# tlog-dev/eazy

Measured on AMD Instinct MI355X. Metric: device-resident compress+decompress GiB/s, 1 MiB block, 1/2/4/8 MI355X, higher is better.
Workload: dtype u8

## Files before the change

### eazy_amd/csrc/ez_k1_lean.hip

```cpp
#include "ez_k1_internal.h"

#include <cstdio>
#include <cstring>
#include <algorithm>
#include <vector>

namespace ez {
namespace {
using namespace k1;

struct GWU {
    const uint8_t *p;
    __device__ __forceinline__ void around(int32_t y, uint64_t &before, uint64_t &from) const {
        V16 v = ld16v(p + (y - 8));
        if (y < 8) {
            const int32_t k = 8 - y;
            v.lo &= k >= 8 ? 0ull : ~0ull << (8 * k);
            v.hi &= k >= 16 ? 0ull : (k <= 8 ? ~0ull : ~0ull << (8 * (k - 8)));
        }
        before = v.lo;
        from = v.hi;
    }
};

template <int R = 80, int G = 16>
struct WinLds {
    static constexpr int LB = 128 / G;
    typedef unsigned int u32v __attribute__((ext_vector_type(LB / 4)));
    u32v f;
    int32_t cb, fb, bmax, pm;
    uint8_t *wl;
    __device__ __forceinline__ int32_t floor4(int32_t y) const { return y - ((pm + y) & 3); }
    __device__ __forceinline__ void ld(const uint8_t *p, int32_t b, int lj, u32v &d) const {
        typedef const __attribute__((address_space(1))) u32v *gp;
        d = *(gp)(p + b + LB * lj);
    }
    __device__ __forceinline__ void put(int lj) const { *(u32v *)(wl + LB * lj) = f; }
    __device__ __forceinline__ void init(const uint8_t *p, int32_t n, int lj, bool live) {
        pm = (int32_t)((uintptr_t)p & 3);
        bmax = floor4(n - 64);
        cb = min(floor4(-8), bmax);
        fb = min(cb + 64, bmax);
        f = u32v{};
        if (live) ld(p, cb, lj, f);
        put(lj);
        if (live) ld(p, fb, lj, f);
    }
    __device__ __forceinline__ void advance(const uint8_t *p, int32_t i, int lj, bool live) {
        const int32_t y = i - 8;
        if (live && !(y >= cb && y - cb <= R)) {
            if (!(y >= fb && y - fb <= R)) {
                fb = min(floor4(y), bmax);
                ld(p, fb, lj, f);
            }
            cb = fb;
            put(lj);
            fb = min(cb + 64, bmax);
            ld(p, fb, lj, f);
        }
    }
    __device__ __forceinline__ void bytes(int32_t i, int g, int lj, V16 &w0, V16 &w1) const {
        const uint32_t o = (uint32_t)(i - 8 - cb + lj), r = o & 3;
        const uint32_t *q = (const uint32_t *)(wl + (o & ~3u));
        uint32_t d[9];
#pragma unroll
        for (int t = 0; t < 9; t++) d[t] = q[t];
        uint32_t b[8];
#pragma unroll
        for (int t = 0; t < 8; t++) b[t] = __builtin_amdgcn_alignbyte(d[t + 1], d[t], r);
        w0.lo = (uint64_t)b[0] | ((uint64_t)b[1] << 32);
        w0.hi = (uint64_t)b[2] | ((uint64_t)b[3] << 32);
        w1.lo = (uint64_t)b[4] | ((uint64_t)b[5] << 32);
        w1.hi = (uint64_t)b[6] | ((uint64_t)b[7] << 32);
    }
    __device__ __forceinline__ void bytes48(int32_t i, int g, int lj, V16 &w0, V16 &w1, V16 &w2) const {
        static_assert(R <= 64, "48-byte windows need the region to reach i + 54");
        const uint32_t o = (uint32_t)(i - 8 - cb + lj), r = o & 3;
        const uint32_t *q = (const uint32_t *)(wl + (o & ~3u));
        uint32_t d[13];
#pragma unroll
        for (int t = 0; t < 13; t++) d[t] = q[t];
        uint32_t b[12];
#pragma unroll
        for (int t = 0; t < 12; t++) b[t] = __builtin_amdgcn_alignbyte(d[t + 1], d[t], r);
        w0 = V16{(uint64_t)b[0] | ((uint64_t)b[1] << 32), (uint64_t)b[2] | ((uint64_t)b[3] << 32)};
        w1 = V16{(uint64_t)b[4] | ((uint64_t)b[5] << 32), (uint64_t)b[6] | ((uint64_t)b[7] << 32)};
        w2 = V16{(uint64_t)b[8] | ((uint64_t)b[9] << 32), (uint64_t)b[10] | ((uint64_t)b[11] << 32)};
    }
};

__device__ __forceinline__ void bytes32(const LeanIn &L, const uint8_t *p, int32_t y, V16 &c0, V16 &c1) {
    const uintptr_t a = (uintptr_t)(p + y - 8);
    const uint32_t r = (uint32_t)(a & 3);
    const uint8_t *w = (const uint8_t *)(a & ~(uintptr_t)3);
    const uint4 q0 = L.dw4(w), q1 = L.dw4(w + 16);
    const uint32_t q2 = L.dw(w + 32);
    const uint32_t d[9] = {q0.x, q0.y, q0.z, q0.w, q1.x, q1.y, q1.z, q1.w, q2};
    uint32_t b[8];
#pragma unroll
    for (int t = 0; t < 8; t++) b[t] = __builtin_amdgcn_alignbyte(d[t + 1], d[t], r);
    c0.lo = (uint64_t)b[0] | ((uint64_t)b[1] << 32);
    c0.hi = (uint64_t)b[2] | ((uint64_t)b[3] << 32);
    c1.lo = (uint64_t)b[4] | ((uint64_t)b[5] << 32);
    c1.hi = (uint64_t)b[6] | ((uint64_t)b[7] << 32);
}

__device__ __forceinline__ void bytes48(const LeanIn &L, const uint8_t *p, int32_t y, V16 &c0, V16 &c1, V16 &c2) {
    const uintptr_t a = (uintptr_t)(p + y);
    const uint32_t r = (uint32_t)(a & 3);
    const uint8_t *w = (const uint8_t *)(a & ~(uintptr_t)3) - 8;
    const uint4 q0 = L.dw4(w), q1 = L.dw4(w + 16), q2 = L.dw4(w + 32);
    const uint32_t q3 = L.dw(w + 48);
    const uint32_t d[13] = {q0.x, q0.y, q0.z, q0.w, q1.x, q1.y, q1.z, q1.w, q2.x, q2.y, q2.z, q2.w, q3};
    uint32_t b[12];
#pragma unroll
    for (int t = 0; t < 12; t++) b[t] = __builtin_amdgcn_alignbyte(d[t + 1], d[t], r);
    c0 = V16{(uint64_t)b[0] | ((uint64_t)b[1] << 32), (uint64_t)b[2] | ((uint64_t)b[3] << 32)};
    c1 = V16{(uint64_t)b[4] | ((uint64_t)b[5] << 32), (uint64_t)b[6] | ((uint64_t)b[7] << 32)};
    c2 = V16{(uint64_t)b[8] | ((uint64_t)b[9] << 32), (uint64_t)b[10] | ((uint64_t)b[11] << 32)};
}

#if (EZ_EXP & 65536)
__device__ unsigned long long g_lean_hist[18];
#endif

template <int FW, int G>
__device__ __forceinline__ void lean_run(const CompressArgs &A, int lj, int g, uint16_t *hth, uint32_t table_words, uint32_t hsh,
                                         uint64_t *recs, uint64_t rcap, int prio, uint8_t *edge, uint8_t *wl) {
    constexpr int S = 64 / G;
    constexpr uint32_t kGMask = (1u << G) - 1;
    constexpr bool W40 = FW == 40;
    static_assert(FW == 24 || W40, "the judgement's forward cap is 24 or 40 bytes");
    constexpr int32_t CAP = FW;
    const LeanIn L{};
    const uint8_t *blo = A.in, *bhi = A.in + A.in_off[A.count];
    uint32_t *slots = (uint32_t *)(edge + 128 + kEdgeSlots * edge_slot_bytes(A));
    const uint32_t rcap32 = (uint32_t)rcap;

    uint64_t s = (uint64_t)blockIdx.x * S + (uint64_t)g;
    const uint8_t *p = edge + 16;
    int32_t n = 0, i = 0, done = 0, nrec = 0;
    int err = 0;
    bool live = false, pending = false;
    uint64_t *rec = recs;
    V16 z0{0, 0}, z1{0, 0}, z2{0, 0};
    WinLds<W40 ? 64 : 80, G> wr;
    wr.wl = wl;
    int64_t budget = 0;

    auto open = [&]() {
        pending = s < A.count;
        n = 0;
        const uint8_t *src = blo;
        if (pending) {
            n = (int32_t)(A.in_off[s + 1] - A.in_off[s]);
            src = A.in + A.in_off[s];
        }
        for (int32_t k = 4 * lj; k < (int32_t)table_words; k += 4 * G) *(uint4 *)((uint32_t *)hth + k) = make_uint4(0, 0, 0, 0);
        err = !pending || (uint64_t)n > A.max_len ? EZ_EINVAL : 0;
        live = !err && n >= 4;
        p = live ? src : edge + 16;
        const bool edge_stream = live && (src - kEdgeBefore < blo || src + n + 64 > bhi);
        if (edge_stream) {
            int32_t slot = 0;
            if (lj == 0) slot = (int32_t)atomicAdd(slots, 1u);
            slot = bcast(slot, G * g);
            if (slot >= kEdgeSlots) {
                err = EZ_ESTUCK;
                live = false;
                p = edge + 16;
            } else {
                uint8_t *d = edge + 128 + (uint64_t)slot * edge_slot_bytes(A);
                for (int32_t k = lj; k < n + kEdgeBefore + 64; k += G)
                    d[k] = (k >= kEdgeBefore && k < n + kEdgeBefore) ? src[k - kEdgeBefore] : (uint8_t)0;
                p = d + kEdgeBefore;
            }
            __threadfence_block();
        }
        i = done = nrec = 0;
        rec = recs + (pending ? s : 0) * rcap;
        wr.init(p, n, lj, live);
        z0 = z1 = z2 = V16{0, 0};
        if (live) {
            if constexpr (W40) bytes48(L, p, 0, z0, z1, z2);
            else bytes32(L, p, 0, z0, z1);
            z0.lo = 0;
        }
    };
    open();
    budget += (int64_t)(4 * A.max_len + 64) * S;

    V16 w0{0, 0}, w1{0, 0}, w2{0, 0};
    for (;;) {
        if (__builtin_amdgcn_ballot_w64(!live && pending) != 0) {
            if (!live && pending) {
                if (lj == 0) A.out_size[s] = (uint64_t)nrec | ((uint64_t)err << 48);
                pending = false;
            }
        }
        if (__builtin_amdgcn_ballot_w64(live) == 0) break;
        if (budget < 0) {
            if (live) err = EZ_ESTUCK;
            live = false;
            continue;
        }
        const uint64_t lm = __builtin_amdgcn_ballot_w64(live);
        do {
        budget--;
        if constexpr (W40) wr.bytes48(i, g, lj, w0, w1, w2);
        else wr.bytes(i, g, lj, w0, w1);
        const int32_t nvalid = n - 3 - i < G ? n - 3 - i : G;
        const int32_t x = i + lj;
        const bool valid = live && lj < nvalid;

        if (prio & 1) __builtin_amdgcn_s_setprio(3);
        const uint32_t h = valid ? ((uint32_t)w0.hi * kHashMul) >> hsh : 0u;
        int32_t cand = 0;
        if (valid) cand = (int32_t)lds_mskor16(hth, h, (uint32_t)x);
        V16 c0 = z0, c1 = z1, c2 = z2;
        if (cand != 0) {
            if constexpr (W40) bytes48(L, p, cand, c0, c1, c2);
            else bytes32(L, p, cand, c0, c1);
            if (__builtin_expect(cand < 8, 0)) c0.lo &= ~0ull << (8 * (8 - cand));
        }
        if (prio & 1) __builtin_amdgcn_s_setprio(0);

        const bool rl = cand >= done && cand < x;
        const uint64_t e0 = w0.hi ^ c0.hi, e1 = w1.lo ^ c1.lo, e2 = w1.hi ^ c1.hi;
        int32_t jf = W40 ? first_diff40(e0, e1, e2, w2.lo ^ c2.lo, w2.hi ^ c2.hi) : first_diff24(e0, e1, e2);
        jf = jf < n - x ? jf : n - x;
        int32_t bl = x - done;
        if (rl) bl = bl < cand ? bl : cand;
        int32_t jb = last_diff8(w0.lo ^ c0.lo);
        jb = jb < bl ? jb : bl;
        const bool zr = rl && c0.hi == 0 && cand + 8 < n;
        const int32_t fw = rl ? jf : (jf < done - cand ? jf : done - cand);
        const bool acc = valid && (zr || fw + jb >= kMinCopyChunk);

        int32_t lit, nx, dist, ext;
        bool force = false;
        if (zr) {
            int32_t zf = W40 ? first_diff40(0, c1.lo, c1.hi, c2.lo, c2.hi) : first_diff24(0, c1.lo, c1.hi);
            zf = zf < n - cand ? zf : n - cand;
            int32_t zb = last_diff8(c0.lo);
            zb = zb < cand - done ? zb : cand - done;
            lit = cand - zb;
            nx = cand + zf;
            dist = 0;
            ext = (zf == CAP && n - cand > CAP ? 1 : 0) | (zb == 8 && cand - done > 8 ? 2 : 0);
        } else {
            lit = x - jb;
            nx = x + fw;
            dist = x - cand;
            force = rl;
            ext = (jf == CAP && (rl ? n - x : (done - cand < n - x ? done - cand : n - x)) > CAP ? 1 : 0) |
                  (jb == 8 && bl > 8 ? 2 : 0);
        }
        const uint64_t am64 = __builtin_amdgcn_ballot_w64(acc);
        const uint32_t am = (uint32_t)(am64 >> (G * g)) & kGMask;
        const int a = am ? __builtin_ctz(am) : -1;
#if (EZ_EXP & 65536)
        if (live && lj == 0) atomicAdd(&g_lean_hist[a + 1], 1ull);
#endif
        const bool act = live && a >= 0;
        const bool ins1 = !rl && !zr && x + 1 + 4 <= n;
        const int32_t pack = nx | (ext << 28) | ((int32_t)ins1 << 30);
        const int32_t sel = __builtin_amdgcn_ds_bpermute(4 * (G * g + (a < 0 ? 0 : a)), pack);
        int32_t nxt = sel & 0x0fffffff;
        if (__builtin_amdgcn_ballot_w64(act && ((sel >> 28) & 3) != 0) != 0) {
            const int32_t info = cand | (((zr ? cand : x) - lit) << 16) | ((int32_t)rl << 29) | ((int32_t)zr << 30);
            const int32_t ib = bcast(info, G * g + (a < 0 ? 0 : a));
            const int32_t xa = i + (a < 0 ? 0 : a);
            const int32_t ca = ib & 0xffff;
            const bool rla = (ib >> 29) & 1, zra = (ib >> 30) & 1;
            const int32_t e = (sel >> 28) & 3;
            const bool need = act && e != 0;
            const int mode = zra ? 0 : (rla ? 1 : 2);
            const int32_t fa = zra ? ca : xa;
            const int32_t blim = zra ? ca - done : (rla ? ((xa - done) < ca ? (xa - done) : ca) : xa - done);
            const int32_t flim = zra ? n - ca : (rla ? n - xa : ((done - ca) < n - xa ? done - ca : n - xa));
            int32_t fx, cx;
            gext<G, GWU>(GWU{p}, need && (e & 1), need && (e & 2), g, lj, fa, ca, mode, done, CAP, flim, blim, fx, cx);
            if (need) {
                const int32_t f = (e & 1) ? fx : (sel & 0x0fffffff) - fa;
                const int32_t c = (e & 2) ? cx : ((ib >> 16) & 0xf);
                nxt = fa + f;
                if (lj == a) {
                    lit = fa - c;
                    nx = nxt;
                }
            }
        }
        const bool ins_next = (prio & 4) && a >= 0 && a < G - 1 && ((sel >> 30) & 1);
        if (valid && a >= 0 && lj > a && cand <= i + a) hth[h] = (uint16_t)(ins_next && lj == a + 1 ? x : cand);
        if (act && lj == a && !ins_next) {
            if (ins1) {
                const uint32_t h1 = ((uint32_t)(w0.hi >> 8) * kHashMul) >> hsh;
                hth[h1] = (uint16_t)(x + 1);
            }
        }
        const bool st_rec = act && lj == a;
        const uint64_t rv = rec_pack(lit, nx - lit, dist, force);
        const uint32_t rat = (uint32_t)nrec;
        const bool rec_room = (uint32_t)nrec < rcap32;
        if (act) {
            if (!rec_room) { err = EZ_ESTUCK; live = false; }
            nrec++;
            i = done = nxt;
        } else if (live) {
            i += nvalid;
        }
        if (live && (err || i + 4 > n)) live = false;
        wr.advance(p, i, lj, live);
        __builtin_amdgcn_sched_barrier(0);
        if (st_rec && rec_room) __builtin_nontemporal_store(rv, rec + rat);
        } while (__builtin_amdgcn_ballot_w64(live) == lm && budget >= 0);
    }
}


constexpr int kLeanWaves16 = 5;
#if (EZ_EXP & 2097152)
constexpr uint32_t kLeanTMax = 1u << 18;
__device__ uint64_t g_lean_t[2 * kLeanTMax];
#endif
template <int FW, int G>
__global__ __launch_bounds__(64, G == 8 ? 2 : kLeanWaves16) void k1_lean(CompressArgs A, uint32_t stride_words, uint32_t table_words, uint64_t *recs,
                                                                          uint64_t rcap, int prio, uint8_t *edge) {
    constexpr int S = 64 / G;
    extern __shared__ __attribute__((aligned(16))) uint8_t smem[];
    const int lane = (int)(threadIdx.x & 63);
    const int g = lane / G, lj = lane % G;
    const int32_t hs = (int32_t)A.hs;
    const uint32_t hsh = 32u - (uint32_t)(64 - __builtin_clzll((uint64_t)(hs - 1)));
    uint16_t *hth = (uint16_t *)((uint32_t *)smem + (uint32_t)g * stride_words);
    uint8_t *wl = smem + (size_t)4 * stride_words * S + (size_t)g * kWinLdsBytes;
#if (EZ_EXP & 2097152)
    const uint64_t t_start = __builtin_amdgcn_s_memrealtime();
#endif
    lean_run<FW, G>(A, lj, g, hth, table_words, hsh, recs, rcap, prio, edge, wl);
#if (EZ_EXP & 2097152)
    {
        const uint64_t t_end = __builtin_amdgcn_s_memrealtime();
        uint32_t hw = 0, xcc = 0;
        asm volatile("s_getreg_b32 %0, hwreg(HW_REG_HW_ID)" : "=s"(hw));
        asm volatile("s_getreg_b32 %0, hwreg(HW_REG_XCC_ID)" : "=s"(xcc));
        if (lane == 0 && blockIdx.x < kLeanTMax) {
            g_lean_t[2 * blockIdx.x] = t_start;
            g_lean_t[2 * blockIdx.x + 1] = (t_end & 0xffffffffffull) | ((uint64_t)((hw >> 8) & 15) << 40) | ((uint64_t)((hw >> 13) & 7) << 44) |
                                           ((uint64_t)((hw >> 12) & 1) << 47) | ((uint64_t)(xcc & 15) << 48) | ((uint64_t)((hw >> 4) & 3) << 52);
        }
    }
#endif
}

#if (EZ_EXP & 2097152)
void lean_report_timeline(uint64_t blocks, hipStream_t st) {
    const uint64_t nb = blocks < kLeanTMax ? blocks : kLeanTMax;
    std::vector<uint64_t> t(2 * nb);
    (void)hipStreamSynchronize(st);
    (void)hipMemcpyFromSymbol(t.data(), HIP_SYMBOL(g_lean_t), 16 * nb);
    uint64_t t0 = ~0ull, t1 = 0, xe[16] = {0}, xs[16], cnt[16] = {0};
    for (int k = 0; k < 16; k++) xs[k] = ~0ull;
    for (uint64_t b = 0; b < nb; b++) {
        const uint64_t st0 = t[2 * b] & 0xffffffffffull, en = t[2 * b + 1] & 0xffffffffffull;
        const int x = (int)((t[2 * b + 1] >> 48) & 15);
        t0 = st0 < t0 ? st0 : t0;
        t1 = en > t1 ? en : t1;
        xe[x] = en > xe[x] ? en : xe[x];
        xs[x] = st0 < xs[x] ? st0 : xs[x];
        cnt[x]++;
    }
    const int bins = 40;
    std::vector<double> act(bins, 0.0);
    std::vector<uint64_t> ends(nb), lens(nb);
    for (uint64_t b = 0; b < nb; b++) {
        const uint64_t st0 = (t[2 * b] & 0xffffffffffull) - t0, en = (t[2 * b + 1] & 0xffffffffffull) - t0;
        ends[b] = en;
        lens[b] = en - st0;
        for (int k = 0; k < bins; k++) {
            const double lo = (double)(t1 - t0) * k / bins, hi = (double)(t1 - t0) * (k + 1) / bins;
            const double ov = std::min((double)en, hi) - std::max((double)st0, lo);
            if (ov > 0) act[k] += ov / (hi - lo);
        }
    }
    std::sort(ends.begin(), ends.end());
    std::sort(lens.begin(), lens.end());
    fprintf(stderr, "lean waves %llu span %.1f us; wave life p10 %.1f p50 %.1f p90 %.1f max %.1f us; end p50 %.1f p90 %.1f p99 %.1f us\n",
            (unsigned long long)nb, (t1 - t0) / 100.0, lens[nb / 10] / 100.0, lens[nb / 2] / 100.0, lens[nb * 9 / 10] / 100.0, lens[nb - 1] / 100.0,
            ends[nb / 2] / 100.0, ends[nb * 9 / 10] / 100.0, ends[nb * 99 / 100] / 100.0);
    fprintf(stderr, "lean active waves per bin of %.1f us:", (t1 - t0) / 100.0 / bins);
    for (int k = 0; k < bins; k++) fprintf(stderr, " %.0f", act[k]);
    fprintf(stderr, "\nlean per xcc (waves, first start, last end, us):");
    for (int x = 0; x < 16; x++)
        if (cnt[x]) fprintf(stderr, " [%d %llu %.1f %.1f]", x, (unsigned long long)cnt[x], (xs[x] - t0) / 100.0, (xe[x] - t0) / 100.0);
    fprintf(stderr, "\n");
}
#endif
#if (EZ_EXP & 65536)
void lean_report_hist(hipStream_t st) {
    unsigned long long hst[18];
    (void)hipStreamSynchronize(st);
    (void)hipMemcpyFromSymbol(hst, HIP_SYMBOL(g_lean_hist), sizeof hst);
    unsigned long long tot = 0, vis = 0;
    for (int t = 0; t < 18; t++) tot += hst[t];
    for (int t = 1; t < 17; t++) vis += hst[t] * (unsigned long long)t;
    vis += hst[0] * 16ull;
    fprintf(stderr, "lean windows %llu (no accept %llu); visited lanes %.3f of 16; by acceptor lane:", tot, hst[0], (double)vis / (double)tot);
    for (int t = 1; t < 17; t++) fprintf(stderr, " %.3f", (double)hst[t] / (double)tot);
    fprintf(stderr, "\n");
    memset(hst, 0, sizeof hst);
    (void)hipMemcpyToSymbol(HIP_SYMBOL(g_lean_hist), hst, sizeof hst);
}
#endif

template <int FW, int G>
hipError_t launch_lean_v(const CompressArgs &a, uint64_t *recs, uint32_t stride, uint32_t tw, size_t lds, int prio, uint8_t *edge,
                         hipStream_t st) {
    static bool attr_done = false;
    if (!attr_done) {
        (void)hipFuncSetAttribute((const void *)k1_lean<FW, G>, hipFuncAttributeMaxDynamicSharedMemorySize, 160 * 1024);
        attr_done = true;
    }
    constexpr uint64_t S = 64 / G;
    const uint64_t blocks = (a.count + S - 1) / S;
    hipLaunchKernelGGL((k1_lean<FW, G>), dim3((unsigned)blocks), dim3(64), lds, st, a, stride, tw, recs, rec_cap(a), prio, edge);
    return hipGetLastError();
}

}

hipError_t launch_lean(const CompressArgs &a, uint64_t *recs, hipStream_t st) {
    const bool g8 = a.max_len > 4096;
    const bool w40 = a.max_len <= 16384;
    const int S = g8 ? 8 : 4;
    const uint32_t stride = split_stride<16, true>(a), tw = split_table_words<true>(a);
    const uint64_t rcap = rec_cap(a);
    static const int prio = knob("EZ_K1S_PRIO", 1) | (knob("EZ_K1S_NEXT1", 1) ? 4 : 0);
    uint8_t *edge = (uint8_t *)(recs + a.count * rcap);
    hipError_t z = hipMemsetAsync(edge, 0, 128, st);
    if (z == hipSuccess) z = hipMemsetAsync(edge + 128 + kEdgeSlots * edge_slot_bytes(a), 0, 16, st);
    if (z != hipSuccess) return z;
    static const size_t pad = (size_t)knob("EZ_K1S_LDSPAD", 0);
    const size_t lds = (size_t)stride * 4 * S + (size_t)kWinLdsBytes * S + pad;
    hipError_t e;
    const char *route;
    if (!g8) route = "s:lean g16 fw40", e = launch_lean_v<40, 16>(a, recs, stride, tw, lds, prio, edge, st);
    else if (w40) route = "s:lean g8 fw40", e = launch_lean_v<40, 8>(a, recs, stride, tw, lds, prio, edge, st);
    else route = "s:lean g8 fw24", e = launch_lean_v<24, 8>(a, recs, stride, tw, lds, prio, edge, st);
    set_compress_route(route);
    if (e != hipSuccess) return e;
#if (EZ_EXP & 2097152)
    lean_report_timeline((a.count + S - 1) / S, st);
#endif
#if (EZ_EXP & 65536)
    lean_report_hist(st);
#endif
    return launch_emit(a, recs, rcap, false, st);
}

}
```

Baseline: 117.1.

## Add interior fast path to lean match loop without bounds checks

Splits the per-window loop body into a templated lambda with an interior variant used while every lane's group has at least G+CAP-1 bytes left and record room. The interior path drops the end-of-block clamps, the liveness and rcap checks, and simplifies the extension flags to fire whenever a match reaches the cap. This is meant to cut scalar and vector ALU work per window in the common case. It adds a wave-wide ballot per iteration and duplicates the loop body, which raises code size and may raise register pressure. It also changes the ext flags in the boundary path, so more gext calls may fire there and rely on flim/blim to stay correct.

```diff
diff --git a/eazy_amd/csrc/ez_k1_lean.hip b/eazy_amd/csrc/ez_k1_lean.hip
--- a/eazy_amd/csrc/ez_k1_lean.hip
+++ b/eazy_amd/csrc/ez_k1_lean.hip
@@ -3,6 +3,7 @@
 #include <cstdio>
 #include <cstring>
 #include <algorithm>
+#include <type_traits>
 #include <vector>
 
 namespace ez {
@@ -121,7 +122,7 @@
 }
 
 #if (EZ_EXP & 65536)
-__device__ unsigned long long g_lean_hist[18];
+__device__ unsigned long long g_lean_hist[23];
 #endif
 
 template <int FW, int G>
@@ -191,27 +192,17 @@
     budget += (int64_t)(4 * A.max_len + 64) * S;
 
     V16 w0{0, 0}, w1{0, 0}, w2{0, 0};
-    for (;;) {
-        if (__builtin_amdgcn_ballot_w64(!live && pending) != 0) {
-            if (!live && pending) {
-                if (lj == 0) A.out_size[s] = (uint64_t)nrec | ((uint64_t)err << 48);
-                pending = false;
-            }
-        }
-        if (__builtin_amdgcn_ballot_w64(live) == 0) break;
-        if (budget < 0) {
-            if (live) err = EZ_ESTUCK;
-            live = false;
-            continue;
-        }
-        const uint64_t lm = __builtin_amdgcn_ballot_w64(live);
-        do {
+
+    constexpr int32_t kIn = G + CAP - 1;
+
+    auto window = [&](auto in_tag) __attribute__((always_inline)) {
+        constexpr bool IN = decltype(in_tag)::value;
         budget--;
         if constexpr (W40) wr.bytes48(i, g, lj, w0, w1, w2);
         else wr.bytes(i, g, lj, w0, w1);
-        const int32_t nvalid = n - 3 - i < G ? n - 3 - i : G;
+        const int32_t nvalid = IN ? G : (n - 3 - i < G ? n - 3 - i : G);
         const int32_t x = i + lj;
-        const bool valid = live && lj < nvalid;
+        const bool valid = IN || (live && lj < nvalid);
 
         if (prio & 1) __builtin_amdgcn_s_setprio(3);
         const uint32_t h = valid ? ((uint32_t)w0.hi * kHashMul) >> hsh : 0u;
@@ -228,12 +219,12 @@
         const bool rl = cand >= done && cand < x;
         const uint64_t e0 = w0.hi ^ c0.hi, e1 = w1.lo ^ c1.lo, e2 = w1.hi ^ c1.hi;
         int32_t jf = W40 ? first_diff40(e0, e1, e2, w2.lo ^ c2.lo, w2.hi ^ c2.hi) : first_diff24(e0, e1, e2);
-        jf = jf < n - x ? jf : n - x;
+        if constexpr (!IN) jf = jf < n - x ? jf : n - x;
         int32_t bl = x - done;
         if (rl) bl = bl < cand ? bl : cand;
         int32_t jb = last_diff8(w0.lo ^ c0.lo);
         jb = jb < bl ? jb : bl;
-        const bool zr = rl && c0.hi == 0 && cand + 8 < n;
+        const bool zr = rl && c0.hi == 0 && (IN || cand + 8 < n);
         const int32_t fw = rl ? jf : (jf < done - cand ? jf : done - cand);
         const bool acc = valid && (zr || fw + jb >= kMinCopyChunk);
 
@@ -241,29 +232,29 @@
         bool force = false;
         if (zr) {
             int32_t zf = W40 ? first_diff40(0, c1.lo, c1.hi, c2.lo, c2.hi) : first_diff24(0, c1.lo, c1.hi);
-            zf = zf < n - cand ? zf : n - cand;
+            if constexpr (!IN) zf = zf < n - cand ? zf : n - cand;
             int32_t zb = last_diff8(c0.lo);
             zb = zb < cand - done ? zb : cand - done;
             lit = cand - zb;
             nx = cand + zf;
             dist = 0;
-            ext = (zf == CAP && n - cand > CAP ? 1 : 0) | (zb == 8 && cand - done > 8 ? 2 : 0);
+            ext = (zf == CAP ? 1 : 0) | (zb == 8 ? 2 : 0);
         } else {
             lit = x - jb;
             nx = x + fw;
             dist = x - cand;
             force = rl;
-            ext = (jf == CAP && (rl ? n - x : (done - cand < n - x ? done - cand : n - x)) > CAP ? 1 : 0) |
-                  (jb == 8 && bl > 8 ? 2 : 0);
+            ext = (jf == CAP ? 1 : 0) | (jb == 8 ? 2 : 0);
         }
         const uint64_t am64 = __builtin_amdgcn_ballot_w64(acc);
         const uint32_t am = (uint32_t)(am64 >> (G * g)) & kGMask;
         const int a = am ? __builtin_ctz(am) : -1;
 #if (EZ_EXP & 65536)
-        if (live && lj == 0) atomicAdd(&g_lean_hist[a + 1], 1ull);
-#endif
-        const bool act = live && a >= 0;
-        const bool ins1 = !rl && !zr && x + 1 + 4 <= n;
+        if ((IN || live) && lj == 0) atomicAdd(&g_lean_hist[a + 1], 1ull);
+        if (lj == 0 && g == 0) atomicAdd(&g_lean_hist[21], 1ull);
+#endif
+        const bool act = (IN || live) && a >= 0;
+        const bool ins1 = !rl && !zr && (IN || x + 1 + 4 <= n);
         const int32_t pack = nx | (ext << 28) | ((int32_t)ins1 << 30);
         const int32_t sel = __builtin_amdgcn_ds_bpermute(4 * (G * g + (a < 0 ? 0 : a)), pack);
         int32_t nxt = sel & 0x0fffffff;
@@ -280,6 +271,11 @@
             const int32_t blim = zra ? ca - done : (rla ? ((xa - done) < ca ? (xa - done) : ca) : xa - done);
             const int32_t flim = zra ? n - ca : (rla ? n - xa : ((done - ca) < n - xa ? done - ca : n - xa));
             int32_t fx, cx;
+#if (EZ_EXP & 65536)
+            if (need && lj == 0) atomicAdd(&g_lean_hist[18 + ((e & 1 && flim > CAP) || (e & 2 && blim > 8) ? 0 : 1)], 1ull);
+            if (lj == 0 && g == 0) atomicAdd(&g_lean_hist[20], 1ull);
+            if (__builtin_amdgcn_ballot_w64(need && ((e & 1 && flim > CAP) || (e & 2 && blim > 8))) != 0 && lj == 0 && g == 0) atomicAdd(&g_lean_hist[22], 1ull);
+#endif
             gext<G, GWU>(GWU{p}, need && (e & 1), need && (e & 2), g, lj, fa, ca, mode, done, CAP, flim, blim, fx, cx);
             if (need) {
                 const int32_t f = (e & 1) ? fx : (sel & 0x0fffffff) - fa;
@@ -302,18 +298,45 @@
         const bool st_rec = act && lj == a;
         const uint64_t rv = rec_pack(lit, nx - lit, dist, force);
         const uint32_t rat = (uint32_t)nrec;
-        const bool rec_room = (uint32_t)nrec < rcap32;
+        const bool rec_room = IN || (uint32_t)nrec < rcap32;
         if (act) {
             if (!rec_room) { err = EZ_ESTUCK; live = false; }
             nrec++;
             i = done = nxt;
-        } else if (live) {
+        } else if (IN || live) {
             i += nvalid;
         }
-        if (live && (err || i + 4 > n)) live = false;
-        wr.advance(p, i, lj, live);
+        if constexpr (!IN) {
+            if (live && (err || i + 4 > n)) live = false;
+        }
+        wr.advance(p, i, lj, IN || live);
         __builtin_amdgcn_sched_barrier(0);
         if (st_rec && rec_room) __builtin_nontemporal_store(rv, rec + rat);
+    };
+
+    for (;;) {
+        if (__builtin_amdgcn_ballot_w64(!live && pending) != 0) {
+            if (!live && pending) {
+                if (lj == 0) A.out_size[s] = (uint64_t)nrec | ((uint64_t)err << 48);
+                pending = false;
+            }
+        }
+        if (__builtin_amdgcn_ballot_w64(live) == 0) break;
+        if (budget < 0) {
+            if (live) err = EZ_ESTUCK;
+            live = false;
+            continue;
+        }
+        if (__builtin_amdgcn_ballot_w64(live && i + kIn <= n && (uint32_t)nrec < rcap32) == ~0ull) {
+            do {
+                window(std::true_type{});
+            } while (__builtin_amdgcn_ballot_w64(i + kIn <= n && (uint32_t)nrec < rcap32) == ~0ull);
+            if (i + 4 > n) live = false;
+            continue;
+        }
+        const uint64_t lm = __builtin_amdgcn_ballot_w64(live);
+        do {
+            window(std::false_type{});
         } while (__builtin_amdgcn_ballot_w64(live) == lm && budget >= 0);
     }
 }
@@ -399,7 +422,7 @@
 #endif
 #if (EZ_EXP & 65536)
 void lean_report_hist(hipStream_t st) {
-    unsigned long long hst[18];
+    unsigned long long hst[23];
     (void)hipStreamSynchronize(st);
     (void)hipMemcpyFromSymbol(hst, HIP_SYMBOL(g_lean_hist), sizeof hst);
     unsigned long long tot = 0, vis = 0;
@@ -408,7 +431,9 @@
     vis += hst[0] * 16ull;
     fprintf(stderr, "lean windows %llu (no accept %llu); visited lanes %.3f of 16; by acceptor lane:", tot, hst[0], (double)vis / (double)tot);
     for (int t = 1; t < 17; t++) fprintf(stderr, " %.3f", (double)hst[t] / (double)tot);
-    fprintf(stderr, "\n");
+    fprintf(stderr, "\nlean capped counts: %llu acceptors with room left, %llu without; gext branch in %llu of %llu wave iterations (%.2f %%), %llu with room left (%.2f %%)\n",
+            hst[18], hst[19], hst[20], hst[21], 100.0 * (double)hst[20] / (double)(hst[21] ? hst[21] : 1), hst[22],
+            100.0 * (double)hst[22] / (double)(hst[21] ? hst[21] : 1));
     memset(hst, 0, sizeof hst);
     (void)hipMemcpyToSymbol(HIP_SYMBOL(g_lean_hist), hst, sizeof hst);
 }
```

Result: faster. 123.7, median of 6 (+5.6%).
